# j-timothy-balint/Metropolis-Hastings-GPGPU

Measured on AMD Instinct MI355X. Metric: MH chain-steps/sec (whole node) + mean final cost, N=64 objects, higher is better.
Workload: dtype f64+f32 (reference precision map)

## Files before the change

metropolis-hastings-gpgpu_amd/csrc/mh_chain.hip:

```cpp

#include <stdint.h>
#include <stdlib.h>

#include "mh_common.h"
#ifndef MH_CHAIN_STEP_TU
#include <rocrand/rocrand_xorwow.h>
#endif
#ifndef MH_DOUBLE
#define MH_DOUBLE 0
#endif
#define MH_REPS(bit) ((MH_DOUBLE & (bit)) ? 2 : 1)
#define MH_CLOBBER() asm volatile("" ::: "memory")
#ifndef MH_STAMPS
#define MH_STAMPS 0
#endif

#if MH_STAMPS
#ifdef MH_CHAIN_STEP_TU
static __device__ unsigned long long g_phase_cycles[16];
#else
__device__ unsigned long long g_phase_cycles[16];
#endif
#define MH_STAMP(t) do { __builtin_amdgcn_sched_barrier(0); asm volatile("s_memtime %0\n\ts_waitcnt lgkmcnt(0)" : "=s"(t) :: "memory"); __builtin_amdgcn_sched_barrier(0); } while (0)
#define MH_PHASE(ch, k, t0) do { unsigned long long _t; MH_STAMP(_t); stage((ch).aux)->cyc[k] += _t - (t0); (t0) = _t; } while (0)
// ... 213 lines not shown
}

template <int L>
__device__ __forceinline__ int inc_cl_update(const ChainPtrs& ch, int n, int c, int ka, int kb,
                                             int r, int gbase, float4 boxj, const ClPairs& clp,
                                             ClPairs& clo, bool& colchg) {
    const int j = r;
    const uint64_t* NZc = ch.NZ.ptr() + clp.buf * c;
    const Staged<uint64_t> NZn = stage(ch.NZ.at((clp.buf ^ 1) * c));
    uint64_t cm = clp.cm;
    uint64_t w = (r < c) ? NZc[r] : 0ull;
    const int kk2[2] = {ka, kb};
#pragma unroll
    for (int q = 0; q < 2; ++q) {
        const int k = kk2[q];
        if (k < 0) continue;
        const ObjP pk = ch.P[k];
        const float4 bk = shape_box(ch.objs[k], pk.xf, pk.yf);
        const bool nzk = r < c && overlap(ch.CLA[r], bk) != 0.0f;
        const uint64_t colk = group_ballot<L>(nzk, gbase);
        if (j == k) cm = colk;
        w = (w & ~(1ull << k)) | ((uint64_t)nzk << k);
    }
    uint64_t moved = group_ballot<L>(r < c && (ch.clrs[r].pad == ka || ch.clrs[r].pad == kb),
                                     gbase);
    while (moved) {
        const int i = __builtin_ctzll(moved);
        moved &= moved - 1;
        const bool nzi = j < n && overlap(ch.CLA[i], boxj) != 0.0f;
        const uint64_t row = group_ballot<L>(nzi, gbase);
        colchg = colchg || nzi || ((cm >> i) & 1ull) != 0;
        cm = (cm & ~(1ull << i)) | ((uint64_t)nzi << i);
        if (r == i) w = row;
    }
    if (r < c) NZn.put(r, w);
    int total;
    const int pre = group_excl_scan<L>(r < c ? __builtin_popcountll(w) : 0, r, total);
    if (r < c) stage(ch.PRE).put(r, pre);
    clo.cm = cm;
    clo.buf = clp.buf ^ 1;
    hand_off(ch.NZ, ch.PRE);
    return total;
}

#ifndef MH_EVAL_INLINE
#define MH_EVAL_INLINE 1
#endif
#if MH_EVAL_INLINE > 0
#define MH_EVAL_ATTR __attribute__((always_inline))
#else
#define MH_EVAL_ATTR __attribute__((noinline))
#endif

template <int L, int NPL, bool WITH_OL, bool DELTA, bool FAST = false, bool PAIRS = false>
__device__ MH_EVAL_ATTR void eval_costs(const LaunchArgs& a, const ChainPtrs& ch, const OwnPose<NPL>& op,
                           int r, int gbase,
                           float out[8], SymRows<NPL>& sym, const SymRows<NPL>& prev, int ka,
                           int kb, ClPairs& clo, const ClPairs& clp, float u_acc = 0.0f,
                           CostIv cur = CostIv{0.0f, 0.0f}, int* fast = nullptr,
                           CostIv* star_iv = nullptr, bool save = false) {
    const DevRoom& rm = PAIRS ? a.rm : *ch.rm;
    const int n = a.rm.n, c = a.rm.c;

    unsigned long long t0 = 0;
    MH_STAMP(t0);
    constexpr bool SHARED = DELTA && NPL == 1 && L >= 16;
    float px[NPL], py[NPL];
    float cph[NPL], rxs[NPL], rys[NPL], rrs[NPL];
    float4 sao[NPL], sac[NPL];
    float4 boxo[NPL];
    double rpw[NPL], rang[NPL];
    bool wild = false;
    for (int rep = 0; rep < MH_REPS(1); ++rep) {
    MH_CLOBBER();
#pragma unroll
    for (int m = 0; m < NPL; ++m) {
        const int i = m * L + r;
        px[m] = py[m] = 0.0f;
        cph[m] = rxs[m] = rys[m] = rrs[m] = 0.0f;
        rpw[m] = rang[m] = 0.0;
        sao[m] = sac[m] = boxo[m] = make_float4(0.f, 0.f, 0.f, 0.f);
        if constexpr (SHARED) {
            const bool moved = i < n && (i == ka || i == kb) && !(MH_ABLATE & 2);
            bool touched = false;
            if (i < rm.r && !(MH_ABLATE & 16)) {
                const uint2 q = ch.rix[i];
                const unsigned a16 = (unsigned)ka, b16 = (unsigned)kb;
                touched = ka >= 0 && ((q.x & 0xffffu) == a16 || (q.x >> 16) == a16 ||
                                      (q.y & 0xffffu) == a16 || (q.y >> 16) == a16 ||
                                      (q.x & 0xffffu) == b16 || (q.x >> 16) == b16 ||
                                      (q.y & 0xffffu) == b16 || (q.y >> 16) == b16);
            }
            cph[m] = clp.cph;
            rpw[m] = clp.rpw;
            rang[m] = clp.rang;
            clo.dc = clp.dc;
            clo.dr = clp.dr;
            clo.eang = clp.eang;
            if constexpr (FAST) {
                bool amb = false, ambo = false;
                if (__ballot(moved || touched))
                    approx_terms<!PAIRS>(ch, rm, i, n, moved, touched, cph[m], rpw[m], rang[m], clo.eang,
                                 amb, ambo);
                clo.dc = clo.dc || moved;
                clo.dr = clo.dr || touched;
                if (__ballot(amb || ambo)) {
                    if (amb) {
// ... 24 lines not shown
            py[m] = (float)vy;
            if (!(MH_ABLATE & 2) && !SHARED) {
                float at = atan2_f32(rm.fyf - p.yf, rm.fxf - p.xf);
                float b = at - p.rotYf;
                float ph = (float)((double)b + kHalfPI);
                cph[m] = cos_f32(ph);
            }
            double al = x * (double)rm.ux;
            al = al + y * (double)rm.uy;
            float sd = (float)(2.0 * (rm.along_f - al));
            rxs[m] = (float)(x + (double)(sd * rm.ux));
            rys[m] = (float)(y + (double)(sd * rm.uy));
            float rr = (float)(rm.two_focal_rot - op.ry[m]);
            if ((double)rr < -kPI) rr = (float)((double)rr + kTwoPI);
            rrs[m] = rr;
            const float4 box = shape_box(os, p.xf, p.yf);
            if constexpr (WITH_OL) stage(ch.OFF).put(i, box);
            sao[m] = comp_overlaps(rm, box);
            boxo[m] = box;
        }
        if constexpr (!SHARED) {
            if (!(MH_ABLATE & 16) && i < rm.r) rel_terms(ch, i, rpw[m], rang[m]);
        }
        if constexpr (NPL == 1) {
            clo.rpw = rpw[0];
            clo.rang = rang[0];
            clo.cph = cph[0];
            if constexpr (!SHARED) {
                clo.dc = clo.dr = false;
                clo.eang = 0.0f;
            }
        }
        if (i < c) {
            const RectShape cs = ch.clrs[i];
            const ObjP ps = ch.P[cs.pad];
            stage(ch.CLA).put(i, shape_box(cs, ps.xf, ps.yf));
        }
        bool sa_new = i < c;
        if constexpr (SHARED) {
            sac[m] = clp.sac;
            sa_new = sa_new && (i == ka || i == kb);
        }
        if (sa_new) {
            const ObjP pi = ch.P[i];
            sac[m] = comp_overlaps(rm, shape_box(ch.clrs[i], pi.xf, pi.yf));
        }
        if constexpr (NPL == 1) clo.sac = sac[0];
    }
    }
    hand_off(ch.PX, ch.PY, ch.CLA, ch.OFF);

    if (r == 0) MH_PHASE(ch, 1, t0);
    const bool exact_mode = group_ballot<L>(wild, gbase) != 0;
    constexpr bool DEFER_SYM = FAST;
    int dlead = -1;
    float esym = 0.0f;
    if constexpr (!DELTA) {
    float m1[NPL], m2[NPL];
    int j1[NPL];
    for (int rep = 0; rep < MH_REPS(2); ++rep) {
    MH_CLOBBER();
#pragma unroll
    for (int m = 0; m < NPL; ++m) {
        m1[m] = m2[m] = -INFINITY;
        j1[m] = -1;
    }
#pragma unroll 2
    for (int j = 0; j < ((MH_ABLATE & 1) ? 0 : n); ++j) {
        const float4 q = objp_f4(ch.P[j]);
#pragma unroll
        for (int m = 0; m < NPL; ++m) {
            const float v = sym_val_fast(q, rxs[m], rys[m], rrs[m]);
            m2[m] = __builtin_amdgcn_fmed3f(m1[m], m2[m], v);
            const bool up = v > m1[m];
            m1[m] = up ? v : m1[m];
            j1[m] = up ? j : j1[m];
        }
    }
    }
    bool amb[NPL];
    bool any_amb = false;
#pragma unroll
    for (int m = 0; m < NPL; ++m) {
        const int i = m * L + r;
        const bool row = i < n;
        const bool clear = j1[m] >= 0 &&
                           (m2[m] == -INFINITY ||
                            m1[m] - m2[m] > sym_err(m1[m], rrs[m]) + sym_err(m2[m], rrs[m]));
        amb[m] = row && (exact_mode || !clear);
        any_amb |= amb[m];
        float e = 0.0f;
        const double ry1 = pose_ry_var<L, NPL>(op, j1[m], gbase);
        if (row && j1[m] >= 0 && MH_CK(j1[m] < n, 7, j1[m], i)) {
            const ObjP q = ch.P[j1[m]];
            e = sym_val_exact(q.xf, q.yf, ry1, rxs[m], rys[m], (double)rrs[m]);
        }
        sym.mx[m] = fmaxf(0.0f, e);
        sym.arg[m] = e > 0.0f ? j1[m] : -1;
    }
    if (__ballot(any_amb)) {
        float thr[NPL];
#pragma unroll
        for (int m = 0; m < NPL; ++m) {
            thr[m] = (exact_mode || j1[m] < 0) ? INFINITY
                                               : 2.0f * sym_err(fabsf(m1[m]) + 1.0f, rrs[m]);
            if (amb[m]) {
                sym.mx[m] = 0.0f;
                sym.arg[m] = -1;
            }
// ... 3 lines not shown
            const double ryj = pose_ry<L, NPL>(op, j, gbase);
#pragma unroll
            for (int m = 0; m < NPL; ++m) {
                if (amb[m]) {
                    const float v = sym_val_fast(objp_f4(q), rxs[m],
                                                 rys[m], rrs[m]);
                    if (!(v < m1[m] - thr[m])) {
                        const float e = sym_val_exact(q.xf, q.yf, ryj, rxs[m], rys[m],
                                                      (double)rrs[m]);
                        if (e > sym.mx[m]) {
                            sym.mx[m] = e;
                            sym.arg[m] = j;
                        }
                    }
                }
            }
        }
    }
    } else {
    bool pairs_done = false;
    if constexpr (PAIRS && L == 64 && NPL == 1) {
        if (n <= 8) {
            const int pi = r >> 3, pj = r & 7;
            const int ai = pi << 2, aj = pj << 2;
            const float prx = __int_as_float(__builtin_amdgcn_ds_bpermute(ai, __float_as_int(rxs[0])));
            const float pry = __int_as_float(__builtin_amdgcn_ds_bpermute(ai, __float_as_int(rys[0])));
            const float prr = __int_as_float(__builtin_amdgcn_ds_bpermute(ai, __float_as_int(rrs[0])));
            const double ryj = __hiloint2double(__builtin_amdgcn_ds_bpermute(aj, __double2hiint(op.ry[0])),
                                                __builtin_amdgcn_ds_bpermute(aj, __double2loint(op.ry[0])));
            const ObjP q = ch.P[pj];
            float v = 0.0f;
            if (pi < n && pj < n)
                v = fmaxf(0.0f, sym_val_exact(q.xf, q.yf, ryj, prx, pry, (double)prr));
            int j = v > 0.0f ? pj : 8;
            group_max_arg<8>(v, j);
            const int src = (r & 7) << 5;
            const float mx = __int_as_float(__builtin_amdgcn_ds_bpermute(src, __float_as_int(v)));
            const int ag = __builtin_amdgcn_ds_bpermute(src, j);
            sym.mx[0] = r < n ? mx : 0.0f;
            sym.arg[0] = (r < n && ag < 8) ? ag : -1;
            pairs_done = true;
        }
    }
    for (int rep = 0; rep < MH_REPS(64) && !pairs_done; ++rep) {
    MH_CLOBBER();
    bool need[NPL];
    unsigned pend[NPL];
    float4 qa = make_float4(0.f, 0.f, 0.f, 0.f), qb = qa;
    if (ka >= 0) qa = objp_f4(ch.P[ka]);
    if (kb >= 0) qb = objp_f4(ch.P[kb]);
    const double rya = pose_ry<L, NPL>(op, ka < 0 ? 0 : ka, gbase);
    const double ryb = pose_ry<L, NPL>(op, kb < 0 ? 0 : kb, gbase);
    bool any_pend = false;
#pragma unroll
    for (int m = 0; m < NPL; ++m) {
        const int i = m * L + r;
        const bool row = i < n;
        const float cm = prev.mx[m];
        const int ca = prev.arg[m];
        sym.mx[m] = cm;
        sym.arg[m] = ca;
        need[m] = row && (i == ka || i == kb);
        pend[m] = 0u;
        if (row && !need[m]) {
            if (ka >= 0) {
                const float v = sym_val_fast(qa, rxs[m], rys[m], rrs[m]);
                const bool below = !exact_mode && v + sym_err(v, rrs[m]) < cm;
                if (ca == ka && below) need[m] = true;
                else if (!below) pend[m] |= 1u;
            }
            if (kb >= 0) {
                const float v = sym_val_fast(qb, rxs[m], rys[m], rrs[m]);
                const bool below = !exact_mode && v + sym_err(v, rrs[m]) < cm;
                if (ca == kb && below) need[m] = true;
                else if (!below) pend[m] |= 2u;
            }
            if (need[m]) pend[m] = 0u;
        }
        any_pend |= pend[m] != 0u;
    }
    while (__ballot(any_pend)) {
        if (any_pend) {
            int ms = NPL - 1;
#pragma unroll
            for (int m = NPL - 2; m >= 0; --m) ms = pend[m] ? m : ms;
            const unsigned pm = sel<NPL>(pend, ms);
            const int col = (pm & 1u) ? ka : kb;
            MH_CK(col >= 0 && col < n, 8, col, pm);
            const ObjP q = ch.P[col];
            const float e = sym_val_exact(q.xf, q.yf, (pm & 1u) ? rya : ryb, sel<NPL>(rxs, ms),
                                          sel<NPL>(rys, ms), (double)sel<NPL>(rrs, ms));
            any_pend = false;
#pragma unroll
            for (int m = 0; m < NPL; ++m) {
                if (m == ms) {
                    pend[m] &= pend[m] - 1u;
                    if (col == prev.arg[m] && !(e >= prev.mx[m])) {
                        need[m] = true;
                    } else if (e > sym.mx[m]) {
                        sym.mx[m] = e;
                        sym.arg[m] = col;
                    }
                }
                any_pend |= pend[m] != 0u;
            }
        }
    }
    uint64_t rows[NPL];
    int lead[NPL];
    unsigned leadp = 0u;
#pragma unroll
    for (int m = 0; m < NPL; ++m) lead[m] = -1;
    bool any_row = false;
#pragma unroll
    for (int m = 0; m < NPL; ++m) {
        rows[m] = group_ballot<L>(need[m], gbase);
        any_row |= rows[m] != 0;
    }
    while (any_row) {
        int ms = NPL - 1;
#pragma unroll
        for (int m = NPL - 2; m >= 0; --m) ms = rows[m] ? m : ms;
        const uint64_t bm = sel<NPL>(rows, ms);
        const int b = __builtin_ctzll(bm);
        const float rx = grp_get<L>(sel<NPL>(rxs, ms), b, gbase);
        const float ry = grp_get<L>(sel<NPL>(rys, ms), b, gbase);
        const float rr = grp_get<L>(sel<NPL>(rrs, ms), b, gbase);
        float t1 = -INFINITY, t2 = -INFINITY;
        int tj = -1;
#pragma unroll
        for (int q = 0; q < NPL; ++q) {
            const int j = q * L + r;
            if (j < n) {
                const float v =
                    sym_val_fast(objp_f4(ch.P[j]), rx, ry, rr);
                t2 = __builtin_amdgcn_fmed3f(t1, t2, v);
                const bool up = v > t1;
                t1 = up ? v : t1;
                tj = up ? j : tj;
            }
        }
        const SymLead ld = group_sym_lead<L>(t1, t2, tj, r, gbase, rr);
        float best = 0.0f;
        int barg = -1;
        const bool clear = !exact_mode && ld.clear;
        if (!clear) {
            const float thr =
                (exact_mode || ld.j < 0) ? INFINITY : 2.0f * sym_err(fabsf(ld.m) + 1.0f, rr);
            float bv = -INFINITY;
            int bj = -1;
#pragma unroll
            for (int q = 0; q < NPL; ++q) {
                const int j = q * L + r;
                if (j >= n) break;
                const ObjP p = ch.P[j];
                const float v = sym_val_fast(objp_f4(p), rx, ry, rr);
                if (!(v < ld.m - thr)) {
                    const float e = sym_val_exact(p.xf, p.yf, op.ry[q], rx, ry, (double)rr);
                    if (e > bv) {
                        bv = e;
                        bj = j;
                    }
                }
            }
            group_max_arg<L>(bv, bj);
            best = bv > 0.0f ? bv : 0.0f;
            barg = bv > 0.0f ? bj : -1;
        }
        any_row = false;
#pragma unroll
        for (int m = 0; m < NPL; ++m) {
            if (m == ms) {
                if (r == b) {
                    if (clear && DEFER_SYM) {
                        dlead = ld.j;
                        esym = sym_err(ld.m, rr);
                        sym.mx[m] = fmaxf(0.0f, ld.m);
                    } else if (clear) {
                        lead[m] = ld.j;
                        leadp |= 1u << m;
                    } else {
                        sym.mx[m] = best;
                        sym.arg[m] = barg;
                    }
                }
                rows[m] &= rows[m] - 1;
            }
            any_row |= rows[m] != 0;
        }
    }
    while (__ballot(leadp != 0u)) {
        const int ms = leadp ? __builtin_ctz(leadp) : 0;
        const int j = leadp ? sel<NPL>(lead, ms) : 0;
        const double ryj = pose_ry_var<L, NPL>(op, j, gbase);
        if (leadp) {
            leadp &= leadp - 1u;
            MH_CK(j >= 0 && j < n, 9, j, ms);
            const ObjP q = ch.P[j];
            const float e = sym_val_exact(q.xf, q.yf, ryj, sel<NPL>(rxs, ms),
                                          sel<NPL>(rys, ms), (double)sel<NPL>(rrs, ms));
#pragma unroll
            for (int m = 0; m < NPL; ++m) {
                if (m == ms) {
                    sym.mx[m] = fmaxf(0.0f, e);
                    sym.arg[m] = e > 0.0f ? j : -1;
                }
            }
        }
    }
    }
    }

    if (r == 0) MH_PHASE(ch, 2, t0);
    constexpr bool INC_CL = DELTA && NPL == 1 && L >= 16;
    int cl_total = 0;
    bool colchg = r < n && (r == ka || r == kb);
    if constexpr (INC_CL) {
#if MH_DOUBLE & 128
        const bool colchg0 = colchg;
        for (int rep = 0; rep < 2; ++rep) {
            MH_CLOBBER();
            colchg = colchg0;
#endif
            cl_total = inc_cl_update<L>(ch, n, c, ka, kb, r, gbase, boxo[0], clp, clo, colchg);
#if MH_DOUBLE & 128
        }
#endif
    }
    if (r == 0) MH_PHASE(ch, 3, t0);
    if constexpr (FAST) {
        static_assert(INC_CL && L == 64, "the rejection bound needs one chain per wavefront");
        if (rm.r <= L) {
            int d = BOUND_OPEN;
#if MH_DOUBLE & 256
            for (int rep = 0; rep < 2; ++rep) {
            MH_CLOBBER();
            float px0 = px[0];
            asm volatile("" : "+v"(px0));
#else
            const float px0 = px[0];
#endif
            float clsum = clp.clc;
            uint64_t bits = r < n ? clo.cm : 0ull;
            const int kcl = __builtin_popcountll(bits);
            if (__ballot(colchg)) {
                if (colchg) {
                    clsum = 0.0f;
                    while (bits) {
                        const int i = __builtin_ctzll(bits);
                        bits &= bits - 1;
                        clsum += overlap(ch.CLA[i], boxo[0]);
                    }
                }
            }
            clo.clc = clsum;
#if MH_CHECK
            {
                float f = 0.0f;
                uint64_t b2 = r < n ? clo.cm : 0ull;
                while (b2) {
                    const int i = __builtin_ctzll(b2);
                    b2 &= b2 - 1;
                    f += overlap(ch.CLA[i], boxo[0]);
                }
                MH_CK(f == clsum, 28, __float_as_uint(f), __float_as_uint(clsum));
            }
#endif
            BoundTerms bt;
            bt.nx = px0;
            bt.ny = py[0];
            bt.anx = fabsf(bt.nx);
            bt.any = fabsf(bt.ny);
            bt.fp = -cph[0];
            bt.afp = fabsf(bt.fp);
            bt.sym = -sym.mx[0];
            bt.symw = r < n ? (float)(n - r) * (sym.mx[0] + esym) : 0.0f;
            bt.esym = esym;
            bt.cl = -clsum;
            bt.kcl = kcl;
            bt.clpos = 0.0f;
            bt.pwd = bt.angd = 0.0;
            bt.efp = r < n && clo.dc ? kDeltaCph : 0.0f;
            bt.eang = r < rm.r && clo.dr ? clo.eang : 0.0f;
            bt.pwx = __ballot(r < rm.r && clo.dr) ? kPwEstU : 0;
            bt.sa = -((sac[0].x + sac[0].y + sac[0].z + sac[0].w) +
                      (sao[0].x + sao[0].y + sao[0].z + sao[0].w));
            bt.pw = -(float)rpw[0];
            bt.ang = -(float)rang[0];
            bt.aang = fabsf(bt.ang);
            bt.k = 8;
            d = bound_decide(rm, n, c, rm.r, cl_total, bt, u_acc, cur, *star_iv, a.bound_slack);
#if MH_DOUBLE & 256
            }
#endif
            if (r == 0) MH_PHASE(ch, 4, t0);
#if MH_STAMPS
            if (r == 0) {
                stage(ch.aux)->cyc[8] += 1;
                stage(ch.aux)->cyc[9] += d == BOUND_REJECT ? 1 : 0;
                stage(ch.aux)->cyc[10] += d == BOUND_ACCEPT ? 1 : 0;
            }
#endif
            if (d == BOUND_REJECT) {
                *fast = d;
                return;
            }
            if constexpr (DEFER_SYM) {
                if (__ballot(dlead >= 0)) {
                    const int j = dlead >= 0 ? dlead : 0;
                    const double ryj = pose_ry_var<L, NPL>(op, j, gbase);
                    if (dlead >= 0) {
                        const ObjP q = ch.P[j];
                        const float e = sym_val_exact(q.xf, q.yf, ryj, rxs[0], rys[0],
                                                      (double)rrs[0]);
                        MH_CK(fabsf(fmaxf(0.0f, e) - sym.mx[0]) <= esym, 33,
                              __float_as_uint(e), __float_as_uint(sym.mx[0]));
                        sym.mx[0] = fmaxf(0.0f, e);
                        sym.arg[0] = e > 0.0f ? j : -1;
                    }
                }
                if (d != BOUND_OPEN) {
                    *fast = d;
                    return;
                }
            }
            const bool obj = r < n && clo.dc, rel = r < rm.r && clo.dr;
            if (__ballot(obj || rel)) {
                float c0 = cph[0];
                double p0 = rpw[0], a0 = rang[0];
                exact_terms(ch, rm, r, n, obj, rel, c0, p0, a0);
#if MH_CHECK
                MH_CK(!obj || fabsf(cph[0] - c0) <= kDeltaCph, 30, __float_as_uint(cph[0]),
                      __float_as_uint(c0));
                MH_CK(!rel || fabs(rpw[0] - p0) <= kPwEstU * 0x1p-24 * fabs(p0) + 1e-30, 31,
                      __float_as_uint((float)rpw[0]), __float_as_uint((float)p0));
                MH_CK(!rel || fabs(rang[0] - a0) <= (double)clo.eang, 32,
                      __float_as_uint((float)rang[0]), __float_as_uint((float)a0));
#endif
                cph[0] = c0;
                rpw[0] = p0;
                rang[0] = a0;
                clo.cph = c0;
                clo.rpw = p0;
                clo.rang = a0;
            }
            clo.dc = clo.dr = false;
            clo.eang = 0.0f;
        }
    }
    double acc = 0.0;
    const bool acc_float = (r == 0 || r == 1 || r == 3 || r == 4);
#pragma unroll
    for (int m = 0; m < NPL; ++m) {
        const int i = m * L + r;
        if (i < n) {
            stage(ch.CPHF).put(i, -cph[m]);
            stage(ch.RMXF).put(i, -sym.mx[m]);
        }
    }
    float sa = 0.0f;
    for (int rep = 0; rep < MH_REPS(4); ++rep) {
    MH_CLOBBER();
    sa = 0.0f;
#pragma unroll
    for (int m = 0; m < NPL; ++m)
        if (m * L < c) sa = serial_sub4<L>(sa, sac[m], gbase);
#pragma unroll
    for (int m = 0; m < NPL; ++m)
        if (m * L < n) sa = serial_sub4<L>(sa, sao[m], gbase);
    }

    int cnt_cl = 0;
    constexpr bool CL_STATE = NPL == 1 && L >= 16;
    bool cl_done = false;
    if constexpr (NPL == 1) {
        const int j = r;
        const float4 boxj = boxo[0];
        if constexpr (INC_CL) {
            const uint64_t* NZn = ch.NZ.ptr() + clo.buf * c;
            if (cl_total <= 2 * L) {
                const uint64_t below = (1ull << j) - 1ull;
                uint64_t bits = j < n ? clo.cm : 0ull;
                while (bits) {
                    const int i = __builtin_ctzll(bits);
                    bits &= bits - 1;
                    const int pos = ch.PRE[i] + __builtin_popcountll(NZn[i] & below);
                    if (MH_CK(i < c && pos >= 0 && pos < 2 * L, 6, i, pos))
                        stage(ch.LCL).put(pos, (double)-overlap(ch.CLA[i], boxj));
                }
                cnt_cl = cl_total;
                cl_done = true;
            }
        } else if constexpr (!DELTA && CL_STATE) {
            uint64_t cm = 0ull;
            float clc = 0.0f;
            for (int i = 0; i < c; ++i) {
                const float ov = j < n ? overlap(ch.CLA[i], boxj) : 0.0f;
                const bool nzi = ov != 0.0f;
                const uint64_t row = group_ballot<L>(nzi, gbase);
                cm |= (uint64_t)nzi << i;
// ... 497 lines not shown
#endif
        Rng rng;
        if constexpr (std::is_same<Rng, WaveRngLds>::value) {
            rng.bsl = reinterpret_cast<float*>(base + F.RNG);
            rng.ss = stage(ch.aux)->rng_key;
        }
        rng_load(rng, a, chain, m0);
        unsigned int accepted = 0;
        float best_total = m0.best_total;
        double beta = kBeta;
        if constexpr (TRACK)
            if (a.n_temps > 1) beta = a.ladder[m0.rung];
        ClPairs cl;
        eval_costs<L, NPL, false, false>(a, ch, op, r, gbase, cur, sym, sym, -1, -1, cl, cl);
#if MH_STAMPS
        if (writer)
            for (int k = 0; k < 12; ++k) stage(ch.aux)->cyc[k] = 0;
        unsigned long long loop_c0 = 0, loop_r0 = 0;
        MH_STAMP(loop_c0);
        asm volatile("s_memrealtime %0\n\ts_waitcnt lgkmcnt(0)" : "=s"(loop_r0) :: "memory");
#endif
#pragma clang loop unroll(disable)
        for (int it = 0; it < a.iterations; ++it) {
            unsigned long long ts = 0;
            MH_STAMP(ts);
            rng_prepare(rng);
            const int2 kk = propose<L, NPL>(rng, OP == OP_STEP_FEW ? a.rm : *rm_l, frozen, ch, op,
                                            r, gbase, writer);
            MH_CK(kk.x < n && kk.y < n && kk.x >= -1 && kk.y >= -1, 11, kk.x, kk.y);
            hand_off(ch.P, ch.aux);
            if (writer) MH_PHASE(ch, 0, ts);
            float sc[8];
            SymRows<NPL> ss;
            ClPairs cls;
            constexpr bool FASTK = !TRACK && FASTK_OF(L, NPL);
            int fast = BOUND_OPEN;
            CostIv star_iv{0.0f, 0.0f};
            float u_acc = 0.0f;
            if constexpr (FASTK) u_acc = rng.uniform();
            eval_costs<L, NPL, false, true, FASTK, OP == OP_STEP_FEW>(
                a, ch, op, r, gbase, sc, ss, sym, kk.x, kk.y, cls, cl, u_acc, cur_iv, &fast,
                &star_iv, true);
            const float star0 = fast != BOUND_OPEN ? 0.0f : L == 64 ? uniform_f(sc[0]) : sc[0];
            MH_STAMP(ts);
#if MH_CHECK
            if constexpr (FASTK)
                if (r == 0) mh_count_decision(fast, true);
            float chk_star = star0;
            if constexpr (FASTK) {
                if (fast != BOUND_OPEN) {
                    float cx[8];
                    SymRows<NPL> sx;
                    ClPairs clx;
                    eval_costs<L, NPL, false, true>(a, ch, op, r, gbase, cx, sx, sym, kk.x, kk.y,
                                                    clx, cl);
                    chk_star = uniform_f(cx[0]);
                    if (r == 0) atomicAdd(&g_check[5], 1u);
                    const bool acc_x =
                        u_acc < accept_threshold(kBeta * ((double)chk_star - (double)chk_cur));
                    if (r == 0) {
                        MH_CK(chk_star >= star_iv.lo && chk_star <= star_iv.hi, 22,
                              __float_as_uint(chk_star), __float_as_uint(star_iv.hi - star_iv.lo));
                        MH_CK(fast != BOUND_REJECT || !acc_x, 20, __float_as_uint(chk_star),
                              __float_as_uint(chk_cur));
                        MH_CK(fast != BOUND_ACCEPT || acc_x, 21, __float_as_uint(chk_star),
                              __float_as_uint(chk_cur));
                    }
                }
                if (r == 0)
                    MH_CK(chk_cur >= cur_iv.lo && chk_cur <= cur_iv.hi, 23,
                          __float_as_uint(chk_cur), __float_as_uint(cur_iv.hi - cur_iv.lo));
            }
#endif
            if constexpr (FASTK) {
                if (__builtin_expect(fast == BOUND_OPEN && !cur_exact, 0)) {
                    const int d2 = decide_exact_star(star0, cur_iv, u_acc, kBeta);
#if MH_CHECK
                    if (r == 0 && d2 != BOUND_OPEN) {
                        const bool acc_x = u_acc < accept_threshold(
                                               kBeta * ((double)star0 - (double)chk_cur));
                        MH_CK(acc_x == (d2 == BOUND_ACCEPT), 25, __float_as_uint(star0),
                              __float_as_uint(chk_cur));
                    }
#endif
                    if (d2 != BOUND_OPEN) fast = d2 + 32;
                }
                if (__builtin_expect(fast == BOUND_OPEN && !cur_exact, 0)) {
                    const int nb = ch.aux->nb;
                    const int k0 = nb > 0 ? ch.aux->b[0].k : 0, k1 = nb > 1 ? ch.aux->b[1].k : 0;
                    MH_CK(nb >= 0 && nb <= 2 && k0 >= 0 && k0 < n && k1 >= 0 && k1 < n, 10,
                          k0 | (nb << 16), k1);
                    const Backup s0 = read_obj<L, NPL>(op, k0, gbase);
                    const Backup s1 = read_obj<L, NPL>(op, k1, gbase);
                    restore<L, NPL>(ch, op, r, writer, kk);
                    hand_off(ch.P, ch.aux);
                    float cx[8];
                    SymRows<NPL> sx;
                    ClPairs clx;
                    eval_costs<L, NPL, false, true>(a, ch, op, r, gbase, cx, sx, ss, kk.x, kk.y, clx,
                                                    cls);
                    if (writer) {
                        const Staged<ChainAux> ax = stage(ch.aux);
                        for (int k = 0; k < 8; ++k) ax->cur[k] = cx[k];
                        if (nb > 0) ax->b[0] = s0;
                        if (nb > 1) ax->b[1] = s1;
                    }
#if MH_STAMPS
                    if (writer) stage(ch.aux)->cyc[11] += 1;
#endif
                    cur_total = uniform_f(cx[0]);
                    cur_exact = true;
                    cur_iv = CostIv{cur_total, cur_total};
#if MH_CHECK
                    if (r == 0) {
                        MH_CK(cur_total == chk_cur, 24, __float_as_uint(cur_total),
                              __float_as_uint(chk_cur));
                        atomicAdd(&g_decide[3], 1ull);
                    }
#endif
                    hand_off(ch.aux);
                    if (u_acc < accept_threshold(kBeta * ((double)star0 - (double)cur_total))) {
                        restore<L, NPL>(ch, op, r, writer, kk);
                        fast = BOUND_ACCEPT + 1;
                    } else {
                        fast = BOUND_REJECT + 16;
                    }
                    hand_off(ch.P);
                }
            }
            if constexpr (TRACK) {
                if (a.track != TRACK_OFF && best_improves(a.track, star0, best_total)) {
                    best_total = star0;
                    save_best_pose<L, NPL>(ch, op, a.best + chain * (int64_t)(F_COUNT * n), n, r);
                }
            }
            bool acc;
            bool exact = true;
            if constexpr (TRACK) acc = accept_at(rng, star0, cur_total, beta);
            else if constexpr (FASTK) {
                if (fast == BOUND_OPEN)
                    acc = u_acc < accept_threshold(kBeta * ((double)star0 - (double)cur_total));
                else
                    acc = fast == BOUND_ACCEPT || fast == BOUND_ACCEPT + 1 ||
                          fast == BOUND_ACCEPT + 32;
                exact = fast != BOUND_ACCEPT;
            } else acc = accept(rng, star0, cur_total);
            if (acc) {
                sym = ss;
                cl = cls;
                ++accepted;
#if MH_CHECK
                if constexpr (FASTK) chk_cur = chk_star;
#endif
                if (exact) {
                    cur_total = star0;
                    if constexpr (FASTK) {
                        cur_exact = true;
                        cur_iv = CostIv{cur_total, cur_total};
                    }
                } else if constexpr (FASTK) {
                    cur_exact = false;
                    cur_iv = star_iv;
                }
                if (writer) {
                    if (exact)
                        for (int k = 0; k < 8; ++k) stage(ch.aux)->cur[k] = ch.aux->star[k];
                    commit_swap_zrr(ch, n);
                }
            } else if (fast != BOUND_REJECT + 16) {
                restore<L, NPL>(ch, op, r, writer, kk);
            }
            hand_off(ch.P, ch.aux);
            if (writer) MH_PHASE(ch, 7, ts);
        }
        if (!cur_exact) {
            float cx[8];
            SymRows<NPL> sx;
            ClPairs clx;
            eval_costs<L, NPL, false, true>(a, ch, op, r, gbase, cx, sx, sym, -1, -1, clx, cl);
            if (writer)
                for (int k = 0; k < 8; ++k) stage(ch.aux)->cur[k] = cx[k];
            hand_off(ch.aux);
        }
#if MH_STAMPS
        if (writer)
            for (int k = 0; k < 12; ++k) atomicAdd(&g_phase_cycles[k], ch.aux->cyc[k]);
        {
            unsigned long long c1 = 0, r1 = 0;
            MH_STAMP(c1);
            asm volatile("s_memrealtime %0\n\ts_waitcnt lgkmcnt(0)" : "=s"(r1) :: "memory");
            if (writer) {
                atomicAdd(&g_phase_cycles[12], c1 - loop_c0);
                atomicAdd(&g_phase_cycles[13], r1 - loop_r0);
            }
        }
#endif
#if MH_CHECK
        if (!TRACK && FASTK_OF(L, NPL) && r == 0)
            MH_CK(ch.aux->cur[0] == chk_cur, 26, __float_as_uint(ch.aux->cur[0]),
                  __float_as_uint(chk_cur));
#endif
        if (writer) {
            ChainMeta m;
            const ChainMeta m1 = a.meta[chain];
            m.accepted = m1.accepted + accepted;
            m.draws = rng_draws(rng);
            m.bm_has = rng.bm_has;
            m.bm_val = rng.bm_val;
            rng_save(rng, a, chain);
            for (int k = 0; k < 8; ++k) m.costs[k] = ch.aux->cur[k];
            m.best_total = TRACK ? best_total : m1.best_total;
            m.rung = m1.rung;
            if (MH_CK(chain >= 0 && chain < a.n_chains, 12, (unsigned)chain, 0)) a.meta[chain] = m;
        }
    } else {
        ClPairs clf;
        MH_CK(a.lay.OFF >= F.end && a.lay.OFF + 16 * n <= a.lay.stride, 16, a.lay.OFF, a.lay.stride);
        eval_costs<L, NPL, true, false>(a, ch, op, r, gbase, cur, sym, sym, -1, -1, clf, clf);
        const int64_t oi = out_index(a, chain);
        const bool oi_ok = MH_CK(oi >= 0 && oi < a.n_chains && oi / a.n_temps == chain / a.n_temps,
                                 14, (unsigned)oi, (unsigned)chain);
        if (r == 0 && oi_ok) {
            resultCosts rc;
            rc.totalCosts = cur[0];
            rc.PairWiseCosts = cur[1];
            rc.VisualBalanceCosts = cur[2];
            rc.FocalPointCosts = cur[3];
            rc.SymmetryCosts = cur[4];
            rc.ClearanceCosts = cur[5];
            rc.OffLimitsCosts = cur[6];
            rc.SurfaceAreaCosts = cur[7];
            a.costs[oi] = rc;
// ... 425 lines not shown
    hipLaunchKernelGGL(mh_summary_kernel, dim3(1), dim3(1024), 0, s, costs, meta, n, chain_offset, out);
    return hipGetLastError();
}

hipError_t launch_suggest_reset(const resultCosts* costs, const point* pts, int64_t n_chains, int n,
                                int group, unsigned char* alive, unsigned long long* keys,
                                int n_keys, float2* xy, hipStream_t s) {
    int64_t work = n_chains * n;
    if (work < n_keys) work = n_keys;
    if (work <= 0) return hipSuccess;
    const int64_t blocks = (work + 255) / 256 < 16384 ? (work + 255) / 256 : 16384;
    hipLaunchKernelGGL(mh_suggest_reset_kernel, dim3((unsigned)blocks), dim3(256), 0, s, costs, pts,
                       n_chains, n, group > 1 ? group : 1, alive, keys, n_keys, xy);
    return hipGetLastError();
}

constexpr int64_t kSuggestBlocks = 2048;

template <int L>
static hipError_t launch_suggest_round_l(const float2* xy, const resultCosts* costs, int64_t n_chains, int n,
                                         const float2* ref, float md2, int64_t kill,
                                         unsigned char* alive, unsigned long long* key,
                                         hipStream_t s) {
    constexpr int G = 256 / L;
    const int64_t passes = (n_chains + G - 1) / G;
    const dim3 grid((unsigned)(passes < kSuggestBlocks ? passes : kSuggestBlocks)), block(256);
    hipLaunchKernelGGL(mh_suggest_round_kernel<L>, grid, block, 0, s, xy, costs, n_chains, n, ref,
                       md2, kill, alive, key);
    return hipGetLastError();
}

hipError_t launch_suggest_round(const float2* xy, const resultCosts* costs,
                                int64_t n_chains, int n, const float2* ref, float md2,
                                int64_t kill, unsigned char* alive, unsigned long long* key,
                                hipStream_t s) {
    if (n_chains <= 0) return hipSuccess;
    if (n_chains >= (1LL << 32) || n < 1) return hipErrorInvalidValue;
    if (n <= 8) return launch_suggest_round_l<8>(xy, costs, n_chains, n, ref, md2, kill, alive, key, s);
    if (n <= 16) return launch_suggest_round_l<16>(xy, costs, n_chains, n, ref, md2, kill, alive, key, s);
    if (n <= 32) return launch_suggest_round_l<32>(xy, costs, n_chains, n, ref, md2, kill, alive, key, s);
    return launch_suggest_round_l<64>(xy, costs, n_chains, n, ref, md2, kill, alive, key, s);
}

#if MH_CHECK
extern "C" __attribute__((visibility("default"))) int mh_debug_check(unsigned int* out) {
    if (hipDeviceSynchronize() != hipSuccess) return -1;
    return hipMemcpyFromSymbol(out, HIP_SYMBOL(g_check), sizeof(unsigned int) * 8) == hipSuccess ? 0 : -1;
}
extern "C" __attribute__((visibility("default"))) int mh_debug_decisions(unsigned long long* out) {
    if (hipDeviceSynchronize() != hipSuccess) return -1;
    return hipMemcpyFromSymbol(out, HIP_SYMBOL(g_decide), sizeof(unsigned long long) * 4) ==
                   hipSuccess ? 0 : -1;
}
#endif

#if MH_STAMPS
extern "C" __attribute__((visibility("default"))) int mh_debug_phase_cycles(unsigned long long* out) {
    if (hipDeviceSynchronize() != hipSuccess) return -1;
    return hipMemcpyFromSymbol(out, HIP_SYMBOL(g_phase_cycles), sizeof(unsigned long long) * 14) ==
                   hipSuccess ? 0 : -1;
}
#endif

hipError_t launch_collectives(int L, const float* v, const int* iv, int* out, hipStream_t s) {
    switch (L) {
        case 8: hipLaunchKernelGGL(mh_collectives_kernel<8>, dim3(1), dim3(64), 0, s, v, iv, out); break;
        case 16: hipLaunchKernelGGL(mh_collectives_kernel<16>, dim3(1), dim3(64), 0, s, v, iv, out); break;
        case 32: hipLaunchKernelGGL(mh_collectives_kernel<32>, dim3(1), dim3(64), 0, s, v, iv, out); break;
        default: hipLaunchKernelGGL(mh_collectives_kernel<64>, dim3(1), dim3(64), 0, s, v, iv, out); break;
    }
    return hipGetLastError();
}

hipError_t launch_rng(int kind, uint64_t seed, uint64_t subsequence, int n, unsigned int* u32,
                      float* uni, float* nrm, hipStream_t s) {
    if (kind == RNG_CURAND_XORWOW)
        hipLaunchKernelGGL(mh_rng_xw_kernel, dim3(1), dim3(64), 0, s, seed, subsequence, n, u32, uni, nrm);
    else
        hipLaunchKernelGGL(mh_rng_kernel, dim3(1), dim3(64), 0, s, seed, subsequence, n, u32, uni, nrm);
    return hipGetLastError();
}

hipError_t launch_math(int fn, uint64_t start, uint64_t count, double* out, hipStream_t s) {
    if (count == 0) return hipSuccess;
    const uint64_t blocks = (count + 255) / 256 < 65536 ? (count + 255) / 256 : 65536;
    hipLaunchKernelGGL(mh_math_kernel, dim3((unsigned)blocks), dim3(256), 0, s, fn, start, count, out);
    return hipGetLastError();
}

hipError_t launch_exchange(const LaunchArgs& a, int* perm, int round, hipStream_t s) {
    const int64_t groups = a.n_chains / a.n_temps;
    if (groups <= 0) return hipSuccess;
    hipLaunchKernelGGL(mh_exchange_kernel, dim3((unsigned)((groups + 255) / 256)), dim3(256), 0, s,
                       a, perm, round);
    return hipGetLastError();
}

hipError_t launch_xorwow_init(uint64_t seed, int64_t chain_offset, int64_t n, unsigned int* xw,
                              hipStream_t s) {
    if (n <= 0) return hipSuccess;
    hipLaunchKernelGGL(mh_xorwow_init_kernel, dim3((unsigned)((n + 255) / 256)), dim3(256), 0, s,
                       seed, chain_offset, n, xw);
    return hipGetLastError();
}

}
// ... 41 lines not shown
```

metropolis-hastings-gpgpu_amd/csrc/mh_common.h:

```cpp
#pragma once

#include <hip/hip_runtime.h>
#include <rocrand/rocrand_philox4x32_10.h>
#include <rocrand/rocrand_uniform.h>

#include <stdint.h>

#include "mh_launch.h"
#include "mh_math.h"

#ifndef MH_ABLATE_OCML
#define MH_ABLATE_OCML 0
#endif
#ifndef MH_ABLATE
#define MH_ABLATE 0
#endif

#ifndef MH_OPT
#define MH_OPT 0
#endif

#ifndef MH_CHECK
#define MH_CHECK 0
#endif
#if MH_CHECK
static __device__ unsigned int g_check[8];
static __device__ unsigned long long g_decide[4];
__device__ __forceinline__ void mh_count_decision(int d, bool evaluated) {
    if (evaluated) atomicAdd(&g_decide[0], 1ull);
    if (d == 1) atomicAdd(&g_decide[1], 1ull);
    if (d == 2) atomicAdd(&g_decide[2], 1ull);
}
__device__ __forceinline__ bool mh_check_fail(unsigned site, unsigned v0, unsigned v1) {
    if (atomicAdd(&g_check[0], 1u) == 0u) {
        g_check[1] = site;
        g_check[2] = v0;
        g_check[3] = v1;
        g_check[4] = blockIdx.x * (blockDim.x >> 6) + (threadIdx.x >> 6);
    }
    return false;
}
#define MH_CK(ok, site, v0, v1) ((ok) ? true : mh_check_fail((site), (unsigned)(v0), (unsigned)(v1)))
#else
#define MH_CK(ok, site, v0, v1) (true)
#endif

namespace mh {

struct alignas(16) ObjP {
    float xf, yf;
    float rotYf;
    float pad;
};

template <class V, class T>
__device__ __forceinline__ V load16(const T* p) {
    static_assert(sizeof(V) == 16, "16-byte loads only");
    V v;
    __builtin_memcpy(&v, __builtin_assume_aligned(p, 16), 16);
    return v;
}
__device__ __forceinline__ float4 objp_f4(const ObjP& p) { return load16<float4>(&p); }


__device__ __forceinline__ void wave_sync() {
    __builtin_amdgcn_fence(__ATOMIC_RELEASE, "wavefront");
    __builtin_amdgcn_wave_barrier();
    __builtin_amdgcn_fence(__ATOMIC_ACQUIRE, "wavefront");
}

template <class T>
struct Published {
    const T* p;
    __device__ __forceinline__ const T& operator[](int i) const { return p[i]; }
    __device__ __forceinline__ const T* ptr() const { return p; }
    __device__ __forceinline__ const T* operator->() const { return p; }
    __device__ __forceinline__ Published<T> at(int off) const { return Published<T>{p + off}; }
};
template <class T>
struct Staged {
// ... 870 lines not shown
    const float t = (o1 + o2) + s_lin;
    const float acur = fmaxf(fabsf(cur.lo), fabsf(cur.hi));
    const float cabs = fabsf(o1) + e1 + fabsf(o2) + e2 + (DPW ? sum[7] : sum[6]);
    e_out = slack * (e1 + e2 + s_elin + 3.0f * U * (fabsf(o1) + fabsf(o2)) +
                     8.0f * U * cabs + 3.0f * U * (fabsf(t) + acur));
    return t;
}

__device__ __forceinline__ int bound_vs(float t, float e, float u, CostIv cur, CostIv& star) {
#pragma clang fp contract(fast)
    const float x = (float)kBeta * ((t + 1.25f * e) - cur.lo);
    const float xl = (float)kBeta * ((t - 1.25f * e) - cur.hi);
    const float lu = __logf(u);
    const bool rej = x <= lu - 1e-4f && x > -1e30f;
    const bool acc = u < 1.0f && (xl >= 0.0f || (xl > -23.9f && lu < xl - 1e-4f));
    star.lo = t - 1.5f * e;
    star.hi = t + 1.5f * e;
    return rej ? BOUND_REJECT : (acc ? BOUND_ACCEPT : BOUND_OPEN);
}

template <bool DPW = false>
__device__ __forceinline__ int bound_compose(const DevRoom& rm, int n, int nrel, int k, int pwx,
                                             const float (&sum)[8], const BoundTerms& bt, float u,
                                             CostIv cur, CostIv& star, float slack) {
    float e;
    const float t = bound_te<DPW>(rm, n, nrel, k, pwx, sum, bt, cur, slack, e);
    return bound_vs(t, e, u, cur, star);
}

template <bool DPW = false>
__device__ __forceinline__ int bound_decide(const DevRoom& rm, int n, int c, int nrel, int ncl,
                                            const BoundTerms& bt, float u, CostIv cur,
                                            CostIv& star, float slack = 1.0f) {
    float part[8], sum[8];
    bound_parts<DPW>(rm, n, c, nrel, ncl, bt, part);
    wave_fsum8(part, sum);
    const int d = bound_compose<DPW>(rm, n, nrel, bt.k, bt.pwx, sum, bt, u, cur, star, slack);
    return __builtin_amdgcn_readfirstlane(d);
}

__device__ __forceinline__ bool certain_reject(const DevRoom& rm, int n, int c, int nrel, int ncl,
                                               const BoundTerms& bt, float u, float cur,
                                               float slack = 1.0f) {
    CostIv star;
    return bound_decide(rm, n, c, nrel, ncl, bt, u, CostIv{cur, cur}, star, slack) ==
           BOUND_REJECT;
}

template <int NPL>
struct SymRows {
    float mx[NPL];
    int arg[NPL];
};

struct ClPairs {
    uint64_t cm;
    int buf;
    double rpw, rang;
    float cph;
    float4 sac;
    bool dc, dr;
    float eang;
    float clc;
};


__device__ __forceinline__ float atan2_est(float y, float x) {
    const float ax = fabsf(x), ay = fabsf(y);
    const float mx = fmaxf(ax, ay), mn = fminf(ax, ay);
    const float t = mn * __builtin_amdgcn_rcpf(mx);
    const float s = t * t;
    float p = -0.0040545351803302765f;
    p = __builtin_fmaf(p, s, 0.021862849593162537f);
    p = __builtin_fmaf(p, s, -0.05591217800974846f);
    p = __builtin_fmaf(p, s, 0.09642186760902405f);
    p = __builtin_fmaf(p, s, -0.1390862613916397f);
    p = __builtin_fmaf(p, s, 0.19946564733982086f);
    p = __builtin_fmaf(p, s, -0.33329859375953674f);
    p = __builtin_fmaf(p, s, 0.9999993443489075f);
    float a = p * t;
    a = ay > ax ? 1.5707963705062866f - a : a;
    a = x < 0.0f ? 3.1415927410125732f - a : a;
    return __builtin_copysignf(a, y);
}

__device__ __forceinline__ float cos_est(float x) {
    const float k = __builtin_rintf(x * 0.63661977236758134f);
    float r = __builtin_fmaf(-k, 1.5707963705062866f, x);
    r = __builtin_fmaf(-k, -4.37113882867379e-08f, r);
    const float s = r * r;
    const float ps = __builtin_fmaf(__builtin_fmaf(s, -0.00019488755788188428f,
                                                   0.008331923745572567f), s, -0.16666649281978607f);
    const float sn = __builtin_fmaf(r * s, ps, r);
    const float pc = __builtin_fmaf(__builtin_fmaf(__builtin_fmaf(s, 2.438225783407688e-05f,
                                                                  -0.0013886678498238325f),
                                                   s, 0.04166661947965622f),
                                    s, -0.5f);
    const float cs = __builtin_fmaf(s, pc, 1.0f);
    const int q = (int)k;
    const float v = (q & 1) ? sn : cs;
    return ((q + 1) & 2) ? -v : v;
}


__device__ __forceinline__ double rel_pw_est(float4 e0, ObjP ps, ObjP pt, bool& amb) {
#pragma clang fp contract(fast)
// ... 168 lines not shown
```

Before: 638.6 million.

## Carry fast-path symmetry row maxima as marked estimates, exactify only when needed

In the fast delta path, each lane's symmetry row maximum can now be stored as an error-bounded fast estimate tagged with a mark bit. This replaces the exact double-precision pending loop and the deferred lead recomputation. The rejection/accept bound uses the estimate plus its error, and exact recomputation runs only when the bound stays open or on non-fast paths (the MARKS template). The aim is to avoid the per-step exact fp64 sym evaluations that steps settled by the bound never need. The cost is more complex state invariants and extra exactify calls on the slow paths.

```diff
diff --git a/metropolis-hastings-gpgpu_amd/csrc/mh_chain.hip b/metropolis-hastings-gpgpu_amd/csrc/mh_chain.hip
--- a/metropolis-hastings-gpgpu_amd/csrc/mh_chain.hip
+++ b/metropolis-hastings-gpgpu_amd/csrc/mh_chain.hip
@@ -289,7 +289,36 @@
 #define MH_EVAL_ATTR __attribute__((noinline))
 #endif
 
-template <int L, int NPL, bool WITH_OL, bool DELTA, bool FAST = false, bool PAIRS = false>
+template <int L, int NPL>
+__device__ __forceinline__ void sym_exactify(const ChainPtrs& ch, const OwnPose<NPL>& op, int gbase,
+                                             int n, float rx, float ry, float rr, float& mx,
+                                             int& arg, bool count) {
+    const bool mk = sym_marked(arg);
+    const uint64_t any = __ballot(mk);
+    if (any) {
+        const int j = sym_col(arg);
+        const double ryj = pose_ry_var<L, NPL>(op, j, gbase);
+        if (mk) {
+            MH_CK(j < n, 9, j, n);
+            const ObjP q = ch.P[j];
+            const float e = sym_val_exact(q.xf, q.yf, ryj, rx, ry, (double)rr);
+            MH_CK(fabsf(fmaxf(0.0f, e) - mx) <= sym_err(mx, rr), 33, __float_as_uint(e),
+                  __float_as_uint(mx));
+            mx = fmaxf(0.0f, e);
+            arg = e > 0.0f ? j : -1;
+        }
+#if MH_CHECK
+        if (count && __lane_id() == (unsigned)__builtin_ctzll(any)) {
+            MH_SYMC(0, 1);
+            MH_SYMC(2, __builtin_popcountll(any));
+            MH_SYMC(3, 1);
+        }
+#endif
+    }
+}
+
+template <int L, int NPL, bool WITH_OL, bool DELTA, bool FAST = false, bool PAIRS = false,
+          int MARKS = 0>
 __device__ MH_EVAL_ATTR void eval_costs(const LaunchArgs& a, const ChainPtrs& ch, const OwnPose<NPL>& op,
                            int r, int gbase,
                            float out[8], SymRows<NPL>& sym, const SymRows<NPL>& prev, int ka,
@@ -420,9 +449,7 @@
 
     if (r == 0) MH_PHASE(ch, 1, t0);
     const bool exact_mode = group_ballot<L>(wild, gbase) != 0;
-    constexpr bool DEFER_SYM = FAST;
-    int dlead = -1;
-    float esym = 0.0f;
+    static_assert(!FAST || (NPL == 1 && MARKS == 0), "marked rows: one object per lane");
     if constexpr (!DELTA) {
     float m1[NPL], m2[NPL];
     int j1[NPL];
@@ -532,15 +559,81 @@
     const double rya = pose_ry<L, NPL>(op, ka < 0 ? 0 : ka, gbase);
     const double ryb = pose_ry<L, NPL>(op, kb < 0 ? 0 : kb, gbase);
     bool any_pend = false;
+    SymRows<NPL> pv = prev;
+    if constexpr (FAST) {
+        const bool row = r < n;
+        float cm = pv.mx[0];
+        bool mk = sym_marked(pv.arg[0]);
+        int ca = sym_col(pv.arg[0]);
+        need[0] = row && (r == ka || r == kb || exact_mode);
+        pend[0] = 0u;
+        bool ovl = false;
+        if (row && !need[0]) {
+            const float rr = rrs[0];
+            float ec = mk ? sym_err(cm, rr) : 0.0f;
+            const int ca0 = ca;
+            if (ka >= 0) {
+                const float v = sym_val_fast(qa, rxs[0], rys[0], rr);
+                const float ev = sym_err(v, rr);
+                const bool held = ka == ca0;
+                if (held ? v - ev >= cm + ec : v - ev > cm + ec) {
+                    cm = v;
+                    ec = ev;
+                    ca = ka;
+                    mk = true;
+                } else if (held) {
+                    need[0] = true;
+                } else if (!(v + ev < cm - ec)) {
+                    ovl = true;
+                }
+            }
+            if (kb >= 0) {
+                const float v = sym_val_fast(qb, rxs[0], rys[0], rr);
+                const float ev = sym_err(v, rr);
+                const bool held = kb == ca0;
+                if (held && ca != ca0) {
+                    need[0] = true;
+                } else if (held ? v - ev >= cm + ec : v - ev > cm + ec) {
+                    cm = v;
+                    ec = ev;
+                    ca = kb;
+                    mk = true;
+                } else if (held) {
+                    need[0] = true;
+                } else if (!(v + ev < cm - ec)) {
+                    ovl = true;
+                }
+            }
+        }
+#if MH_CHECK
+        if (const uint64_t ob = __ballot(ovl && !need[0]); ob && r == __builtin_ctzll(ob))
+            MH_SYMC(1, __builtin_popcountll(ob));
+#endif
+        need[0] = need[0] || ovl;
+        sym.mx[0] = cm;
+        sym.arg[0] = mk ? (ca | kSymMark) : ca;
+    } else {
+    if constexpr (MARKS != 0) {
+        static_assert(NPL == 1, "marked rows: one object per lane");
+        const int lc = sym_col(pv.arg[0]);
+        const bool redo = sym_marked(pv.arg[0]) && (r == ka || r == kb || lc == ka || lc == kb);
+        if (redo) {
+            pv.mx[0] = 0.0f;
+            pv.arg[0] = -1;
+        }
+        sym_exactify<L, NPL>(ch, op, gbase, n, rxs[0], rys[0], rrs[0], pv.mx[0], pv.arg[0],
+                             MARKS == 1);
+        need[0] = redo;
+    }
 #pragma unroll
     for (int m = 0; m < NPL; ++m) {
         const int i = m * L + r;
         const bool row = i < n;
-        const float cm = prev.mx[m];
-        const int ca = prev.arg[m];
+        const float cm = pv.mx[m];
+        const int ca = pv.arg[m];
         sym.mx[m] = cm;
         sym.arg[m] = ca;
-        need[m] = row && (i == ka || i == kb);
+        need[m] = row && (i == ka || i == kb || (MARKS != 0 && need[m]));
         pend[m] = 0u;
         if (row && !need[m]) {
             if (ka >= 0) {
@@ -559,7 +652,8 @@
         }
         any_pend |= pend[m] != 0u;
     }
-    while (__ballot(any_pend)) {
+    }
+    while (!FAST && __ballot(any_pend)) {
         if (any_pend) {
             int ms = NPL - 1;
 #pragma unroll
@@ -575,7 +669,7 @@
             for (int m = 0; m < NPL; ++m) {
                 if (m == ms) {
                     pend[m] &= pend[m] - 1u;
-                    if (col == prev.arg[m] && !(e >= prev.mx[m])) {
+                    if (col == pv.arg[m] && !(e >= pv.mx[m])) {
                         need[m] = true;
                     } else if (e > sym.mx[m]) {
                         sym.mx[m] = e;
@@ -623,8 +717,16 @@
         const SymLead ld = group_sym_lead<L>(t1, t2, tj, r, gbase, rr);
         float best = 0.0f;
         int barg = -1;
-        const bool clear = !exact_mode && ld.clear;
+        const float es = sym_err(ld.m, rr);
+        const bool clear =
+            !exact_mode && ld.clear && !(FAST && !(ld.m - es > 0.0f) && !(ld.m + es <= 0.0f));
         if (!clear) {
+#if MH_CHECK
+            if (FAST && r == b) {
+                MH_SYMC(0, 1);
+                MH_SYMC(1, 1);
+            }
+#endif
             const float thr =
                 (exact_mode || ld.j < 0) ? INFINITY : 2.0f * sym_err(fabsf(ld.m) + 1.0f, rr);
             float bv = -INFINITY;
@@ -652,10 +754,10 @@
         for (int m = 0; m < NPL; ++m) {
             if (m == ms) {
                 if (r == b) {
-                    if (clear && DEFER_SYM) {
-                        dlead = ld.j;
-                        esym = sym_err(ld.m, rr);
-                        sym.mx[m] = fmaxf(0.0f, ld.m);
+                    if (FAST && clear) {
+                        const bool pos = ld.m - es > 0.0f;
+                        sym.mx[m] = pos ? ld.m : 0.0f;
+                        sym.arg[m] = pos ? (ld.j | kSymMark) : -1;
                     } else if (clear) {
                         lead[m] = ld.j;
                         leadp |= 1u << m;
@@ -669,7 +771,7 @@
             any_row |= rows[m] != 0;
         }
     }
-    while (__ballot(leadp != 0u)) {
+    while (!FAST && __ballot(leadp != 0u)) {
         const int ms = leadp ? __builtin_ctz(leadp) : 0;
         const int j = leadp ? sel<NPL>(lead, ms) : 0;
         const double ryj = pose_ry_var<L, NPL>(op, j, gbase);
@@ -710,6 +812,27 @@
     if (r == 0) MH_PHASE(ch, 3, t0);
     if constexpr (FAST) {
         static_assert(INC_CL && L == 64, "the rejection bound needs one chain per wavefront");
+#if MH_CHECK
+        {
+            float fresh = -INFINITY, el = 0.0f;
+            const int lj = sym_col(sym.arg[0]);
+            for (int j = 0; j < n; ++j) {
+                const double ryj = pose_ry<L, NPL>(op, j, gbase);
+                const ObjP q = ch.P[j];
+                const float e = sym_val_exact(q.xf, q.yf, ryj, rxs[0], rys[0], (double)rrs[0]);
+                fresh = fmaxf(fresh, e);
+                el = j == lj ? e : el;
+            }
+            if (r < n && sym_marked(sym.arg[0])) {
+                MH_CK(fabsf(fmaxf(0.0f, el) - sym.mx[0]) <= sym_err(sym.mx[0], rrs[0]), 33,
+                      __float_as_uint(el), __float_as_uint(sym.mx[0]));
+                MH_CK(el == fresh && el > 0.0f, 34, __float_as_uint(el), __float_as_uint(fresh));
+            } else if (r < n) {
+                MH_CK(sym.mx[0] == fmaxf(0.0f, fresh), 35, __float_as_uint(sym.mx[0]),
+                      __float_as_uint(fresh));
+            }
+        }
+#endif
         if (rm.r <= L) {
             int d = BOUND_OPEN;
 #if MH_DOUBLE & 256
@@ -746,6 +869,7 @@
                 MH_CK(f == clsum, 28, __float_as_uint(f), __float_as_uint(clsum));
             }
 #endif
+            const float esym = sym_marked(sym.arg[0]) ? sym_err(sym.mx[0], rrs[0]) : 0.0f;
             BoundTerms bt;
             bt.nx = px0;
             bt.ny = py[0];
@@ -781,29 +905,12 @@
                 stage(ch.aux)->cyc[10] += d == BOUND_ACCEPT ? 1 : 0;
             }
 #endif
-            if (d == BOUND_REJECT) {
+            if (d != BOUND_OPEN) {
                 *fast = d;
                 return;
             }
-            if constexpr (DEFER_SYM) {
-                if (__ballot(dlead >= 0)) {
-                    const int j = dlead >= 0 ? dlead : 0;
-                    const double ryj = pose_ry_var<L, NPL>(op, j, gbase);
-                    if (dlead >= 0) {
-                        const ObjP q = ch.P[j];
-                        const float e = sym_val_exact(q.xf, q.yf, ryj, rxs[0], rys[0],
-                                                      (double)rrs[0]);
-                        MH_CK(fabsf(fmaxf(0.0f, e) - sym.mx[0]) <= esym, 33,
-                              __float_as_uint(e), __float_as_uint(sym.mx[0]));
-                        sym.mx[0] = fmaxf(0.0f, e);
-                        sym.arg[0] = e > 0.0f ? j : -1;
-                    }
-                }
-                if (d != BOUND_OPEN) {
-                    *fast = d;
-                    return;
-                }
-            }
+            sym_exactify<L, NPL>(ch, op, gbase, n, rxs[0], rys[0], rrs[0], sym.mx[0], sym.arg[0],
+                                 true);
             const bool obj = r < n && clo.dc, rel = r < rm.r && clo.dr;
             if (__ballot(obj || rel)) {
                 float c0 = cph[0];
@@ -826,6 +933,9 @@
             }
             clo.dc = clo.dr = false;
             clo.eang = 0.0f;
+        } else {
+            sym_exactify<L, NPL>(ch, op, gbase, n, rxs[0], rys[0], rrs[0], sym.mx[0], sym.arg[0],
+                                 true);
         }
     }
     double acc = 0.0;
@@ -1429,8 +1539,8 @@
                     float cx[8];
                     SymRows<NPL> sx;
                     ClPairs clx;
-                    eval_costs<L, NPL, false, true>(a, ch, op, r, gbase, cx, sx, sym, kk.x, kk.y,
-                                                    clx, cl);
+                    eval_costs<L, NPL, false, true, false, false, 2>(a, ch, op, r, gbase, cx, sx,
+                                                                     sym, kk.x, kk.y, clx, cl);
                     chk_star = uniform_f(cx[0]);
                     if (r == 0) atomicAdd(&g_check[5], 1u);
                     const bool acc_x =
@@ -1444,6 +1554,7 @@
                               __float_as_uint(chk_cur));
                     }
                 }
+                MH_CK(!cur_exact || !sym_marked(sym.arg[0]), 36, sym.arg[0], r);
                 if (r == 0)
                     MH_CK(chk_cur >= cur_iv.lo && chk_cur <= cur_iv.hi, 23,
                           __float_as_uint(chk_cur), __float_as_uint(cur_iv.hi - cur_iv.lo));
@@ -1472,10 +1583,9 @@
                     restore<L, NPL>(ch, op, r, writer, kk);
                     hand_off(ch.P, ch.aux);
                     float cx[8];
-                    SymRows<NPL> sx;
                     ClPairs clx;
-                    eval_costs<L, NPL, false, true>(a, ch, op, r, gbase, cx, sx, ss, kk.x, kk.y, clx,
-                                                    cls);
+                    eval_costs<L, NPL, false, true>(a, ch, op, r, gbase, cx, sym, ss, kk.x, kk.y,
+                                                    clx, cls);
                     if (writer) {
                         const Staged<ChainAux> ax = stage(ch.aux);
                         for (int k = 0; k < 8; ++k) ax->cur[k] = cx[k];
@@ -1554,7 +1664,8 @@
             float cx[8];
             SymRows<NPL> sx;
             ClPairs clx;
-            eval_costs<L, NPL, false, true>(a, ch, op, r, gbase, cx, sx, sym, -1, -1, clx, cl);
+            eval_costs<L, NPL, false, true, false, false, (!TRACK && FASTK_OF(L, NPL)) ? 1 : 0>(
+                a, ch, op, r, gbase, cx, sx, sym, -1, -1, clx, cl);
             if (writer)
                 for (int k = 0; k < 8; ++k) stage(ch.aux)->cur[k] = cx[k];
             hand_off(ch.aux);
@@ -2086,6 +2197,11 @@
     return hipMemcpyFromSymbol(out, HIP_SYMBOL(g_decide), sizeof(unsigned long long) * 4) ==
                    hipSuccess ? 0 : -1;
 }
+extern "C" __attribute__((visibility("default"))) int mh_debug_symrows(unsigned long long* out) {
+    if (hipDeviceSynchronize() != hipSuccess) return -1;
+    return hipMemcpyFromSymbol(out, HIP_SYMBOL(g_symc), sizeof(unsigned long long) * 4) ==
+                   hipSuccess ? 0 : -1;
+}
 #endif
 
 #if MH_STAMPS
diff --git a/metropolis-hastings-gpgpu_amd/csrc/mh_common.h b/metropolis-hastings-gpgpu_amd/csrc/mh_common.h
--- a/metropolis-hastings-gpgpu_amd/csrc/mh_common.h
+++ b/metropolis-hastings-gpgpu_amd/csrc/mh_common.h
@@ -26,6 +26,8 @@
 #if MH_CHECK
 static __device__ unsigned int g_check[8];
 static __device__ unsigned long long g_decide[4];
+static __device__ unsigned long long g_symc[4];
+#define MH_SYMC(k, v) atomicAdd(&g_symc[(k)], (unsigned long long)(v))
 __device__ __forceinline__ void mh_count_decision(int d, bool evaluated) {
     if (evaluated) atomicAdd(&g_decide[0], 1ull);
     if (d == 1) atomicAdd(&g_decide[1], 1ull);
@@ -1002,6 +1004,9 @@
     float mx[NPL];
     int arg[NPL];
 };
+constexpr int kSymMark = 0x40000000;
+__device__ __forceinline__ bool sym_marked(int arg) { return arg >= kSymMark; }
+__device__ __forceinline__ int sym_col(int arg) { return arg < 0 ? -1 : (arg & (kSymMark - 1)); }
 
 struct ClPairs {
     uint64_t cm;
```

Result: faster. 647.8 million, median of 6 (+1.4%).
